# acoustic-warfare/zybo-rt-sampler-image-detection

Measured on AMD Instinct MI355X. Metric: beam-steered frames/sec (64 mics x 256 samples x 101x101 angles), higher is better.
Workload: dtype f32

## Files before the change

zybo-rt-sampler-image-detection_amd/csrc/das_kernels.hip:

```cpp
#include "das_kernels.h"

#include <algorithm>
#include <type_traits>

namespace bf {

namespace {

constexpr int kWave = 64;

struct KArgs {
    long long miso_row;
    int n_mics, m_total, n_samples, n_taps;
    int dir_begin, dir_end, image_stride, image_origin;
    int lead, row_stride, mic_chunk, n_chunks, tile_dirs, n_tiles;
    int scratch_off, srow, pbw;
    int n_is_pow2;
    float inv_n;
    int n_frames;
    int wg_frames, frame_inner;
    long long digest_h_off;
    long long digest_t_off;
};

// ... 1387 lines not shown
    const int f1 = two ? f0 + 1 : f0;
    const int tile_begin = a.dir_begin + tile * a.tile_dirs;
    if (tile_begin >= a.dir_end) return;
    const int tile_end = min(tile_begin + a.tile_dirs, a.dir_end);
    const int M = a.n_mics, N = a.n_samples;
    const int n_half = M / HC;
    const float* __restrict__ sig0 = signals + (size_t)f0 * a.m_total * N;
    const float* __restrict__ sig1 = signals + (size_t)f1 * a.m_total * N;
    float* __restrict__ img0 = images + (size_t)f0 * a.image_stride;
    float* __restrict__ img1 = images + (size_t)f1 * a.image_stride;
    const int32_t* __restrict__ dig = reinterpret_cast<const int32_t*>(taps);

    const int vmic = (lane < n_half) ? mics[lane * HC + (wave >> 1)] : 0;
    auto fetch = [&](int h) -> float4 {
        const int mic = (h < kWave) ? __builtin_amdgcn_readlane(vmic, h) : mics[h * HC + (wave >> 1)];
        const float* src = ((wave & 1) ? sig1 : sig0) + (size_t)mic * N;
        float4 v = make_float4(0.f, 0.f, 0.f, 0.f);
        if (4 * lane < N) v = *reinterpret_cast<const float4*>(src + 4 * lane);
        return v;
    };
    auto stage = [&](int h, const float4 v, bool wipe) {
        float* row0 = lds + (((h & 1) * W) + wave) * G::kSlot;
        const float py = dpp_prev(v.y), pz = dpp_prev(v.z), pw = dpp_prev(v.w);
        write_copies<C>(row0, RS, LEAD, lane, v, py, pz, pw);
        if (wipe) {
            static_assert((LEAD >> 2) * C <= kWave, "one lane per prefix quad");
            constexpr int PQ = LEAD >> 2;
            if (lane < PQ * C) reinterpret_cast<float4*>(row0 + (lane / PQ) * RS)[lane % PQ] = make_float4(0.f, 0.f, 0.f, 0.f);
        }
    };

    float4 st = fetch(0);
    const int lb = 16 * lane + (int)(unsigned)(size_t)((__attribute__((address_space(3))) char*)lds);
    BF_STAMP_DECL

    for (int g0 = tile_begin; g0 < tile_end; g0 += kGroup) {
        f32x2 acc[DW][2][2];
#pragma unroll
        for (int j = 0; j < DW; ++j)
#pragma unroll
            for (int f = 0; f < 2; ++f) { acc[j][f][0] = f32x2{0.0f, 0.0f}; acc[j][f][1] = f32x2{0.0f, 0.0f}; }

        BF_STAMP(7);
        __syncthreads();
        BF_STAMP(1);
        stage(0, st, true);
        st = fetch(1);
        BF_STAMP(2);
        __syncthreads();
        BF_STAMP(3);

        for (int h = 0; h < n_half; ++h) {
            if (h + 1 < n_half) {
                stage(h + 1, st, h == 0);
                if (h + 2 < n_half) st = fetch(h + 2);
                else if (g0 + kGroup < tile_end) st = fetch(0);
                BF_STAMP(2);
            }
            const int dw0 = g0 + wave * DW;
            if (dw0 < tile_end) {
                const size_t grp = (size_t)(dw0 - a.dir_begin) / DW;
                const int32_t* __restrict__ et = dig + (grp * M + (size_t)h * HC) * DW;
                struct Entries { int e[DW]; };
                auto request = [&](Entries& t, int m) {
#pragma unroll
                    for (int j = 0; j < DW; ++j) t.e[j] = et[m * DW + j];
                };
                Entries E[3];
                Quad S0, S1;
                S0.lo = S0.hi = S1.lo = S1.hi = f32x2{0.0f, 0.0f};
                request(E[0], 0);
                request(E[1], 1);
                auto mic = [&](int m, auto kc) {
                    constexpr int K = decltype(kc)::value, K2 = (K + 2) % 3;
                    const Entries& cur = E[K];
                    pair_pad_first(acc, S0, S1, cur.e[0], cur.e[1], lb);
                    request(E[K2], m + 2);
                    pair_pad_rest(acc, S0, S1, cur.e, lb);
                };
                using I0 = std::integral_constant<int, 0>; using I1 = std::integral_constant<int, 1>; using I2 = std::integral_constant<int, 2>;
                static_assert(HC == 8, "eight mics: two trips of three and two more");
#pragma unroll 1
                for (int t = 0; t < 2; ++t) {
                    mic(0, I0{}); mic(1, I1{}); mic(2, I2{});
                    et += 3 * DW;
                }
                mic(0, I0{});
                mic(1, I1{});
            }
            BF_STAMP(0);
            __syncthreads();
            BF_STAMP(h + 1 < n_half ? 3 : 4);
        }

#pragma unroll
        for (int f = 0; f < 2; ++f) {
            if (f == 1) {
                __syncthreads();
                BF_STAMP(4);
            }
            auto park = [&](auto mul_c) {
#pragma unroll
                for (int j = 0; j < DW; ++j) {
                    float* row = lds + (wave * DW + j) * kPark;
                    const f32x2 a0 = acc[j][f][0], a1 = acc[j][f][1];
                    float o0, o1, o2, o3;
                    if constexpr (decltype(mul_c)::value) {
                        o0 = a0.x * a.inv_n; o1 = a0.y * a.inv_n; o2 = a1.x * a.inv_n; o3 = a1.y * a.inv_n;
                    } else {
                        float fm = (float)M;
                        asm volatile("" : "+v"(fm));
                        o0 = a0.x / fm; o1 = a0.y / fm; o2 = a1.x / fm; o3 = a1.y / fm;
                    }
                    reinterpret_cast<float4*>(row)[lane] = make_float4(o0 * o0, o1 * o1, o2 * o2, o3 * o3);
                }
            };
            if (__builtin_expect(a.n_is_pow2, 1)) park(std::true_type{}); else park(std::false_type{});
            BF_STAMP(5);
            __syncthreads();
            BF_STAMP(6);
            const int g = wave * kWave + lane;
            const int d = g0 + g;
            if (g < kGroup && d < tile_end && (f == 0 || two)) {
                const float* row = lds + g * kPark;
                const float4* row4 = reinterpret_cast<const float4*>(row);
                float sum = 0.0f;
                int k = 0;
                for (; k + 32 <= N; k += 32) {
                    float4 v[8];
#pragma unroll
                    for (int u = 0; u < 8; ++u) v[u] = row4[(k >> 2) + u];
#pragma unroll
                    for (int u = 0; u < 8; ++u) { sum += v[u].x; sum += v[u].y; sum += v[u].z; sum += v[u].w; }
                }
                for (; k < N; ++k) sum += row[k];
                (f == 0 ? img0 : img1)[d - a.image_origin] = sum / (float)N;
            }
        }
    }
    BF_STAMP(7);
    BF_STAMP_FLUSH;
}
#undef BF_P_ACC
#undef BF_P_PAD_STEP
#undef BF_P_PAD_READ
#undef BF_P_ADDR
#undef BF_P_CHECK
#undef BF_P_STUB

struct Pair2Geo {
    static constexpr int kC = 2, kLead = Geo<1>::kLead, kRs = 2 * Geo<1>::kRs, kMc = 16, kHalf = 8;
    static constexpr int kSlot = 2 * kC * kRs;
    static constexpr int kDoff = kC * kRs * 4;
};

#define BF_I_ACC(n, j) [a##n##0] "+v"(acc[j][0]), [a##n##1] "+v"(acc[j][1]), [a##n##2] "+v"(acc[j][2]), [a##n##3] "+v"(acc[j][3])
#define BF_I_READ                                                                                   \
    "ds_read_b128 v[96:99], v120\n\tds_read_b128 v[100:103], v120 offset:1024\n\t"                   \
    "ds_read_b128 v[104:107], v120 offset:%[g0]\n\tds_read_b128 v[108:111], v120 offset:%[g1]\n\ts_waitcnt lgkmcnt(0)\n\t"
#define BF_I_STEP(n, h, mods)                                                                       \
    "v_pk_fma_f32 v[112:113], %[" #h "], v[104:105], v[96:97] " mods "\n\tv_pk_fma_f32 v[114:115], %[" #h "], v[106:107], v[98:99] " mods "\n\t" \
    "v_pk_fma_f32 v[116:117], %[" #h "], v[108:109], v[100:101] " mods "\n\tv_pk_fma_f32 v[118:119], %[" #h "], v[110:111], v[102:103] " mods "\n\t" \
    "v_pk_add_f32 %[a" #n "0], %[a" #n "0], v[112:113]\n\tv_pk_add_f32 %[a" #n "1], %[a" #n "1], v[114:115]\n\t" \
    "v_pk_add_f32 %[a" #n "2], %[a" #n "2], v[116:117]\n\tv_pk_add_f32 %[a" #n "3], %[a" #n "3], v[118:119]\n\t"
#define BF_I_FIRST(h, mods)                                                                         \
    "ds_read_b128 v[96:99], v120\n\tds_read_b128 v[104:107], v120 offset:%[g0]\n\t"                \
    "ds_read_b128 v[100:103], v120 offset:1024\n\tds_read_b128 v[108:111], v120 offset:%[g1]\n\ts_waitcnt lgkmcnt(2)\n\t" \
    "v_pk_fma_f32 v[112:113], %[" #h "], v[104:105], v[96:97] " mods "\n\tv_pk_fma_f32 v[114:115], %[" #h "], v[106:107], v[98:99] " mods "\n\t" \
    "v_pk_add_f32 %[a00], %[a00], v[112:113]\n\tv_pk_add_f32 %[a01], %[a01], v[114:115]\n\ts_waitcnt lgkmcnt(0)\n\t" \
    "v_pk_fma_f32 v[116:117], %[" #h "], v[108:109], v[100:101] " mods "\n\tv_pk_fma_f32 v[118:119], %[" #h "], v[110:111], v[102:103] " mods "\n\t" \
    "v_pk_add_f32 %[a02], %[a02], v[116:117]\n\tv_pk_add_f32 %[a03], %[a03], v[118:119]\n\t"
#define BF_I_EVEN "op_sel_hi:[0,1,1]"
#define BF_I_ODD "op_sel:[1,0,0] op_sel_hi:[1,1,1]"
#define BF_I_CHECK(n, ep, ec) "s_cmp_lg_u32 %[" #ec "], %[" #ep "]\n\ts_cbranch_scc1 .Lr" #n "_%=\n.Lb" #n "_%=:\n\t"
#define BF_I_STUB(n, ec) ".Lr" #n "_%=:\n\tv_add_u32 v120, %[" #ec "], %[lb]\n\t" BF_I_READ "s_branch .Lb" #n "_%=\n"
#define BF_I_CLOB "v96", "v97", "v98", "v99", "v100", "v101", "v102", "v103", "v104", "v105", "v106", "v107", "v108", "v109", "v110", "v111", "v112", \
                  "v113", "v114", "v115", "v116", "v117", "v118", "v119", "v120"

__device__ __forceinline__ void pair2_first(f32x2 (&acc)[8][4], int e0, unsigned long long h01, int lbase)
{
    using G = Pair2Geo;
    asm volatile("v_add_u32 v120, %[e0], %[lb]\n\t" BF_I_FIRST(h01, BF_I_EVEN) ";BF_S1_END"
                 : BF_I_ACC(0, 0) : [e0] "s"(e0), [h01] "s"(h01), [lb] "v"(lbase), [g0] "n"(G::kDoff), [g1] "n"(G::kDoff + 1024) : BF_I_CLOB);
}
__device__ __forceinline__ void pair2_rest(f32x2 (&acc)[8][4], const int (&e)[8], const unsigned long long (&hp)[4], int lbase)
{
    using G = Pair2Geo;
    asm volatile(";BF_S2_BEGIN\n\t"
                 BF_I_CHECK(1, e0, e1) BF_I_STEP(1, h01, BF_I_ODD) BF_I_CHECK(2, e1, e2) BF_I_STEP(2, h23, BF_I_EVEN)
                 BF_I_CHECK(3, e2, e3) BF_I_STEP(3, h23, BF_I_ODD) BF_I_CHECK(4, e3, e4) BF_I_STEP(4, h45, BF_I_EVEN)
                 BF_I_CHECK(5, e4, e5) BF_I_STEP(5, h45, BF_I_ODD) BF_I_CHECK(6, e5, e6) BF_I_STEP(6, h67, BF_I_EVEN)
                 BF_I_CHECK(7, e6, e7) BF_I_STEP(7, h67, BF_I_ODD)
                 ".subsection 1\n" BF_I_STUB(1, e1) BF_I_STUB(2, e2) BF_I_STUB(3, e3) BF_I_STUB(4, e4) BF_I_STUB(5, e5) BF_I_STUB(6, e6) BF_I_STUB(7, e7)
                 "\t.subsection 0"
                 : BF_I_ACC(1, 1), BF_I_ACC(2, 2), BF_I_ACC(3, 3), BF_I_ACC(4, 4), BF_I_ACC(5, 5), BF_I_ACC(6, 6), BF_I_ACC(7, 7)
                 : [e0] "s"(e[0]), [e1] "s"(e[1]), [e2] "s"(e[2]), [e3] "s"(e[3]), [e4] "s"(e[4]), [e5] "s"(e[5]), [e6] "s"(e[6]), [e7] "s"(e[7]), [lb] "v"(lbase),
                   [h01] "s"(hp[0]), [h23] "s"(hp[1]), [h45] "s"(hp[2]), [h67] "s"(hp[3]), [g0] "n"(G::kDoff), [g1] "n"(G::kDoff + 1024)
                 : "scc", BF_I_CLOB);
}
#undef BF_I_ACC
#undef BF_I_READ
#undef BF_I_FIRST
#undef BF_I_STEP
#undef BF_I_EVEN
#undef BF_I_ODD
#undef BF_I_CHECK
#undef BF_I_STUB
#undef BF_I_CLOB

template <int ALGO>
__global__ void __launch_bounds__(1024, 4) das_pair2_kernel(BF_TABLE_PARAMS, KArgs a)
{
    static_assert(ALGO == ALGO_LERP, "das_pair2_kernel: lerp (pad runs das_pair_kernel)");
    using G = Pair2Geo;
    constexpr int C = G::kC, RS = G::kRs, LEAD = G::kLead, HC = G::kHalf, W = 16, DW = 8, kGroup = DW * W, kPark = Geo<1>::kPark;
    extern __shared__ __attribute__((aligned(16))) float lds[];
    const int lane_ = threadIdx.x & (kWave - 1), lane = lane_;
    const int wave = __builtin_amdgcn_readfirstlane((int)(threadIdx.x >> 6));
    int tile, fpair;
    tile_and_frame(a, &tile, &fpair);
    const int f0 = 2 * fpair;
    const bool two = f0 + 1 < a.n_frames;
    const int f1 = two ? f0 + 1 : f0;
    const int tile_begin = a.dir_begin + tile * a.tile_dirs;
    if (tile_begin >= a.dir_end) return;
    const int tile_end = min(tile_begin + a.tile_dirs, a.dir_end);
    const int M = a.n_mics, N = a.n_samples;
    const int n_half = M / HC;
    const float* __restrict__ sig0 = signals + (size_t)f0 * a.m_total * N;
    const float* __restrict__ sig1 = signals + (size_t)f1 * a.m_total * N;
    float* __restrict__ img0 = images + (size_t)f0 * a.image_stride;
    float* __restrict__ img1 = images + (size_t)f1 * a.image_stride;
    const int32_t* __restrict__ dig = reinterpret_cast<const int32_t*>(taps);

    const int my_mic = wave & 7, part = wave >> 3;
    const int vmic = (lane < n_half) ? mics[lane * HC + my_mic] : 0;
    struct Staged2 { float4 v0, v1; };
    auto fetch = [&](int h) -> Staged2 {
        const int mic = (h < kWave) ? __builtin_amdgcn_readlane(vmic, h) : mics[h * HC + my_mic];
        Staged2 st;
        st.v0 = make_float4(0.f, 0.f, 0.f, 0.f);
        st.v1 = st.v0;
        if (4 * lane < N) {
            unsigned voff = 16u * (unsigned)lane;
            asm volatile("" : "+v"(voff));
            const char* r0 = reinterpret_cast<const char*>(sig0 + (size_t)mic * N);
            const char* r1 = reinterpret_cast<const char*>(sig1 + (size_t)mic * N);
            st.v0 = *reinterpret_cast<const float4*>(r0 + voff);
            st.v1 = *reinterpret_cast<const float4*>(r1 + voff);
        }
        return st;
    };
    auto write_row = [&](float* row, const float4 x0, const float4 x1, float p0, float p1, bool shifted, int lane) {
        float4* q = reinterpret_cast<float4*>(row + 2 * LEAD) + 2 * lane;
        if (!shifted) {
            q[0] = make_float4(x0.x, x1.x, x0.y, x1.y);
            q[1] = make_float4(x0.z, x1.z, x0.w, x1.w);
        } else {
            q[0] = make_float4(p0, p1, x0.x, x1.x);
            q[1] = make_float4(x0.y, x1.y, x0.z, x1.z);
        }
    };
    auto stage = [&](int h, const Staged2& st, bool wipe) {
        int lane = lane_;
        asm volatile("" : "+v"(lane));
        float* slot = lds + ((h & 1) * HC + my_mic) * G::kSlot;
        float4 x0 = st.v0, x1 = st.v1;
        float* rows = slot + part * C * RS;
        if (part == 1) {
            const float n0 = dpp_next(x0.x), n1 = dpp_next(x1.x);
            x0 = make_float4(x0.y - x0.x, x0.z - x0.y, x0.w - x0.z, n0 - x0.w);
            x1 = make_float4(x1.y - x1.x, x1.z - x1.y, x1.w - x1.z, n1 - x1.w);
        }
        const float p0 = dpp_prev(x0.w), p1 = dpp_prev(x1.w);
        write_row(rows, x0, x1, p0, p1, false, lane);
        write_row(rows + RS, x0, x1, p0, p1, true, lane);
        if (wipe) {
            constexpr int PQ = LEAD >> 1;
            static_assert(2 * PQ <= kWave, "one lane per prefix quad of two rows");
            if (lane < 2 * PQ) reinterpret_cast<float4*>(rows + (lane / PQ) * RS)[lane % PQ] = make_float4(0.f, 0.f, 0.f, 0.f);
        }
    };

    BF_STAMP_DECL
    Staged2 st = fetch(0);
    const int lb = 16 * lane + (int)(unsigned)(size_t)((__attribute__((address_space(3))) char*)lds);

    for (int g0 = tile_begin; g0 < tile_end; g0 += kGroup) {
        f32x2 acc[DW][4];
#pragma unroll
        for (int j = 0; j < DW; ++j)
#pragma unroll
            for (int q = 0; q < 4; ++q) acc[j][q] = f32x2{0.0f, 0.0f};

        BF_STAMP(7);
        __syncthreads();
        BF_STAMP(1);
        stage(0, st, true);
        st = fetch(1 % n_half);
        BF_STAMP(2);
        __syncthreads();
        BF_STAMP(3);

        const int dw0 = g0 + wave * DW;
        const bool busy = dw0 < tile_end;
        const size_t grp = busy ? (size_t)(dw0 - a.dir_begin) / DW : 0;
        for (int h = 0; h < n_half; ++h) {
            if (h + 1 < n_half) {
                stage(h + 1, st, h == 0);
                if (h + 2 < n_half) st = fetch(h + 2);
                else if (g0 + kGroup < tile_end) st = fetch(0);
                BF_STAMP(2);
            }
            if (busy) {
                const int32_t* __restrict__ et = dig + (grp * M + (size_t)h * HC) * DW;
                const float* __restrict__ ht = reinterpret_cast<const float*>(dig) + a.digest_h_off + (grp * M + (size_t)h * HC) * DW;
                struct Entries { int e[DW]; unsigned long long hp[DW / 2]; };
                auto request = [&](Entries& t, int m) {
#pragma unroll
                    for (int j = 0; j < DW; ++j) t.e[j] = et[m * DW + j];
#pragma unroll
                    for (int j = 0; j < DW / 2; ++j) t.hp[j] = *reinterpret_cast<const unsigned long long*>(ht + m * DW + 2 * j);
                };
                Entries E[3];
                request(E[0], 0);
                request(E[1], 1);
                auto mic = [&](int m, auto kc) {
                    constexpr int K = decltype(kc)::value, K2 = (K + 2) % 3;
                    const Entries& cur = E[K];
                    pair2_first(acc, cur.e[0], cur.hp[0], lb);
                    request(E[K2], m + 2);
                    pair2_rest(acc, cur.e, cur.hp, lb);
                };
                using I0 = std::integral_constant<int, 0>; using I1 = std::integral_constant<int, 1>; using I2 = std::integral_constant<int, 2>;
                static_assert(HC == 8, "eight mics: two trips of three and two more");
#pragma unroll 1
                for (int t = 0; t < 2; ++t) {
                    mic(0, I0{}); mic(1, I1{}); mic(2, I2{});
                    et += 3 * DW; ht += 3 * DW;
                }
                mic(0, I0{});
                mic(1, I1{});
                __builtin_amdgcn_s_waitcnt(0xC07F);
            }
            BF_STAMP(0);
            __syncthreads();
            BF_STAMP(h + 1 < n_half ? 3 : 4);
        }

#pragma unroll
        for (int f = 0; f < 2; ++f) {
            if (f == 1) {
                __syncthreads();
                BF_STAMP(4);
            }
            auto park = [&](auto mul_c) __attribute__((always_inline)) {
#pragma unroll
                for (int j = 0; j < DW; ++j) {
                    float* row = lds + (wave * DW + j) * kPark;
                    const float x0 = f == 0 ? acc[j][0].x : acc[j][0].y, x1 = f == 0 ? acc[j][1].x : acc[j][1].y;
                    const float x2 = f == 0 ? acc[j][2].x : acc[j][2].y, x3 = f == 0 ? acc[j][3].x : acc[j][3].y;
                    float o0, o1, o2, o3;
                    if constexpr (decltype(mul_c)::value) {
                        o0 = x0 * a.inv_n; o1 = x1 * a.inv_n; o2 = x2 * a.inv_n; o3 = x3 * a.inv_n;
                    } else {
                        float fm = (float)M;
                        asm volatile("" : "+v"(fm));
                        o0 = x0 / fm; o1 = x1 / fm; o2 = x2 / fm; o3 = x3 / fm;
                    }
                    reinterpret_cast<float2*>(row)[lane] = make_float2(o0 * o0, o1 * o1);
                    reinterpret_cast<float2*>(row + 128)[lane] = make_float2(o2 * o2, o3 * o3);
                }
            };
            if (__builtin_expect(a.n_is_pow2, 1)) park(std::true_type{}); else park(std::false_type{});
            BF_STAMP(5);
            __syncthreads();
            BF_STAMP(6);
            int lane_o = lane;
            asm volatile("" : "+v"(lane_o));
            const int g = wave * kWave + lane_o;
            const int d = g0 + g;
            if (g < kGroup && d < tile_end && (f == 0 || two)) {
                const float* row = lds + g * kPark;
                const float4* row4 = reinterpret_cast<const float4*>(row);
                float sum = 0.0f;
                int k = 0;
                for (; k + 32 <= N; k += 32) {
                    float4 v[8];
#pragma unroll
                    for (int u = 0; u < 8; ++u) v[u] = row4[(k >> 2) + u];
#pragma unroll
                    for (int u = 0; u < 8; ++u) { sum += v[u].x; sum += v[u].y; sum += v[u].z; sum += v[u].w; }
                }
                for (; k < N; ++k) sum += row[k];
                (f == 0 ? img0 : img1)[d - a.image_origin] = sum / (float)N;
            }
        }
    }
    BF_STAMP(7);
    BF_STAMP_FLUSH;
}

struct HybridGeo {
    static constexpr int kC = 2, kLead = Geo<1>::kLead, kRs = 2 * Geo<1>::kRsFir;
    static constexpr int kHalf = 16, kMc = 2 * kHalf;
    static constexpr int kSlot = kC * kRs;
};

struct HybridMasks { unsigned long long m[4]; };
#define BF_H_MASKS                                                                                          \
    "s_lshl_b64 %[m0], -1, %[ng]\n\t"                                                                       \
    "s_lshr_b32 %[t], %[ng], 8\n\ts_lshl_b64 %[m1], -1, %[t]\n\t"                                            \
    "s_lshr_b32 %[t], %[ng], 16\n\ts_lshl_b64 %[m2], -1, %[t]\n\t"                                           \
    "s_lshr_b32 %[t], %[ng], 24\n\ts_lshl_b64 %[m3], -1, %[t]\n\t"
#define BF_H_READS                                                                                          \
    "ds_read_b128 %[q0], %[ad] offset:0\n\tds_read_b128 %[q1], %[ad] offset:16\n\tds_read_b128 %[q2], %[ad] offset:32\n\t" \
    "ds_read_b128 %[q3], %[ad] offset:48\n\tds_read_b128 %[q4], %[ad] offset:64\n\tds_read_b128 %[q5], %[ad] offset:80\n\t"
#define BF_H_QOPS [q0] "+v"(Q[0]), [q1] "+v"(Q[1]), [q2] "+v"(Q[2]), [q3] "+v"(Q[3]), [q4] "+v"(Q[4]), [q5] "+v"(Q[5])
__device__ __forceinline__ void hybrid_window(f32x4 (&Q)[6], HybridMasks& k, int ep, int ec, int ng, int lbase)
{
    int ad, t;
    asm volatile("s_cmp_lg_u32 %[ec], %[ep]\n\ts_cbranch_scc1 .Lr_%=\n.Lb_%=:\n\t"
                 ".subsection 1\n.Lr_%=:\n\tv_add_u32 %[ad], %[ec], %[lb]\n\t" BF_H_READS BF_H_MASKS
                 "s_waitcnt lgkmcnt(0)\n\ts_branch .Lb_%=\n\t.subsection 0"
                 : BF_H_QOPS, [ad] "=&v"(ad), [m0] "+s"(k.m[0]), [m1] "+s"(k.m[1]), [m2] "+s"(k.m[2]), [m3] "+s"(k.m[3]), [t] "=&s"(t)
                 : [ep] "s"(ep), [ec] "s"(ec), [ng] "s"(ng), [lb] "v"(lbase)
                 : "scc");
}
__device__ __forceinline__ void hybrid_window_first(f32x4 (&Q)[6], HybridMasks& k, int ec, int ng, int lbase)
{
    int ad, t;
    asm volatile("v_add_u32 %[ad], %[ec], %[lb]\n\t" BF_H_READS BF_H_MASKS "s_waitcnt lgkmcnt(0)"
                 : BF_H_QOPS, [ad] "=&v"(ad), [m0] "=&s"(k.m[0]), [m1] "=&s"(k.m[1]), [m2] "=&s"(k.m[2]), [m3] "=&s"(k.m[3]), [t] "=&s"(t)
                 : [ec] "s"(ec), [ng] "s"(ng), [lb] "v"(lbase)
                 : "scc");
}
#undef BF_H_MASKS
#undef BF_H_READS
#undef BF_H_QOPS

#define BF_H_E(j, hh, w) "v_pk_fma_f32 %[o" #j "], %[" #hh "], %[w" #w "], %[o" #j "] op_sel_hi:[0,1,1]\n\t"
#define BF_H_O(j, hh, w) "v_pk_fma_f32 %[o" #j "], %[" #hh "], %[w" #w "], %[o" #j "] op_sel:[1,0,0] op_sel_hi:[1,1,1]\n\t"
#define BF_H_OUT(j, w0, w1, w2, w3, w4, w5, w6, w7)                                                          \
    BF_H_E(j, h01, w0) BF_H_O(j, h01, w1) BF_H_E(j, h23, w2) BF_H_O(j, h23, w3) BF_H_E(j, h45, w4) BF_H_O(j, h45, w5) BF_H_E(j, h67, w6) BF_H_O(j, h67, w7)
__device__ __forceinline__ void hybrid_step(f32x2 (&o)[4], const f32x4 (&Q)[6], const unsigned long long (&h)[4], const HybridMasks& k)
{
    const f32x2 w0 = __builtin_shufflevector(Q[0], Q[0], 0, 1), w1 = __builtin_shufflevector(Q[0], Q[0], 2, 3);
    const f32x2 w2 = __builtin_shufflevector(Q[1], Q[1], 0, 1), w3 = __builtin_shufflevector(Q[1], Q[1], 2, 3);
    const f32x2 w4 = __builtin_shufflevector(Q[2], Q[2], 0, 1), w5 = __builtin_shufflevector(Q[2], Q[2], 2, 3);
    const f32x2 w6 = __builtin_shufflevector(Q[3], Q[3], 0, 1), w7 = __builtin_shufflevector(Q[3], Q[3], 2, 3);
    const f32x2 w8 = __builtin_shufflevector(Q[4], Q[4], 0, 1), w9 = __builtin_shufflevector(Q[4], Q[4], 2, 3);
    const f32x2 w10 = __builtin_shufflevector(Q[5], Q[5], 0, 1);
    asm volatile(
        "s_mov_b64 exec, %[m0]\n\t"
        BF_H_OUT(0, 0, 1, 2, 3, 4, 5, 6, 7)
        "s_mov_b64 exec, %[m1]\n\t"
        BF_H_OUT(1, 1, 2, 3, 4, 5, 6, 7, 8)
        "s_mov_b64 exec, %[m2]\n\t"
        BF_H_OUT(2, 2, 3, 4, 5, 6, 7, 8, 9)
        "s_mov_b64 exec, %[m3]\n\t"
        BF_H_OUT(3, 3, 4, 5, 6, 7, 8, 9, 10)
        "s_mov_b64 exec, -1"
        : [o0] "+v"(o[0]), [o1] "+v"(o[1]), [o2] "+v"(o[2]), [o3] "+v"(o[3])
        : [h01] "s"(h[0]), [h23] "s"(h[1]), [h45] "s"(h[2]), [h67] "s"(h[3]), [m0] "s"(k.m[0]), [m1] "s"(k.m[1]), [m2] "s"(k.m[2]), [m3] "s"(k.m[3]),
          [w0] "v"(w0), [w1] "v"(w1), [w2] "v"(w2), [w3] "v"(w3), [w4] "v"(w4), [w5] "v"(w5), [w6] "v"(w6), [w7] "v"(w7), [w8] "v"(w8), [w9] "v"(w9),
          [w10] "v"(w10));
}
__device__ __forceinline__ void fir_naive_step(f32x2 (&o)[4], const f32x4 (&Q)[6], const unsigned long long (&h)[4])
{
    const f32x2 w0 = __builtin_shufflevector(Q[0], Q[0], 0, 1), w1 = __builtin_shufflevector(Q[0], Q[0], 2, 3);
    const f32x2 w2 = __builtin_shufflevector(Q[1], Q[1], 0, 1), w3 = __builtin_shufflevector(Q[1], Q[1], 2, 3);
    const f32x2 w4 = __builtin_shufflevector(Q[2], Q[2], 0, 1), w5 = __builtin_shufflevector(Q[2], Q[2], 2, 3);
    const f32x2 w6 = __builtin_shufflevector(Q[3], Q[3], 0, 1), w7 = __builtin_shufflevector(Q[3], Q[3], 2, 3);
    const f32x2 w8 = __builtin_shufflevector(Q[4], Q[4], 0, 1), w9 = __builtin_shufflevector(Q[4], Q[4], 2, 3);
    const f32x2 w10 = __builtin_shufflevector(Q[5], Q[5], 0, 1);
    asm volatile(
        BF_H_OUT(0, 0, 1, 2, 3, 4, 5, 6, 7) BF_H_OUT(1, 1, 2, 3, 4, 5, 6, 7, 8) BF_H_OUT(2, 2, 3, 4, 5, 6, 7, 8, 9) BF_H_OUT(3, 3, 4, 5, 6, 7, 8, 9, 10)
        : [o0] "+v"(o[0]), [o1] "+v"(o[1]), [o2] "+v"(o[2]), [o3] "+v"(o[3])
        : [h01] "s"(h[0]), [h23] "s"(h[1]), [h45] "s"(h[2]), [h67] "s"(h[3]),
          [w0] "v"(w0), [w1] "v"(w1), [w2] "v"(w2), [w3] "v"(w3), [w4] "v"(w4), [w5] "v"(w5), [w6] "v"(w6), [w7] "v"(w7), [w8] "v"(w8), [w9] "v"(w9),
          [w10] "v"(w10));
}
#define BF_V_MUL(p, hh, w, MODS) "v_pk_mul_f32 %[" #p "], %[" #hh "], %[w" #w "] " MODS "\n\t"
#define BF_V_OUT(j, w0, w1, w2, w3, w4, w5, w6, w7)                                                                             \
    BF_V_MUL(p0, h01, w0, "op_sel_hi:[0,1]") BF_V_MUL(p1, h01, w1, "op_sel:[1,0] op_sel_hi:[1,1]")                                \
    BF_V_MUL(p2, h23, w2, "op_sel_hi:[0,1]") BF_V_MUL(p3, h23, w3, "op_sel:[1,0] op_sel_hi:[1,1]")                                \
    BF_V_MUL(p4, h45, w4, "op_sel_hi:[0,1]") BF_V_MUL(p5, h45, w5, "op_sel:[1,0] op_sel_hi:[1,1]")                                \
    BF_V_MUL(p6, h67, w6, "op_sel_hi:[0,1]") BF_V_MUL(p7, h67, w7, "op_sel:[1,0] op_sel_hi:[1,1]")                                \
    "v_pk_add_f32 %[p0], %[p0], %[p4]\n\tv_pk_add_f32 %[p1], %[p1], %[p5]\n\tv_pk_add_f32 %[p2], %[p2], %[p6]\n\tv_pk_add_f32 %[p3], %[p3], %[p7]\n\t" \
    "v_pk_add_f32 %[p0], %[p0], %[p2]\n\tv_pk_add_f32 %[p1], %[p1], %[p3]\n\tv_pk_add_f32 %[p0], %[p0], %[p1]\n\t"                   \
    "v_pk_add_f32 %[o" #j "], %[o" #j "], %[p0]\n\t"
__device__ __forceinline__ void fir_vec_step(f32x2 (&o)[4], const f32x4 (&Q)[6], const unsigned long long (&h)[4])
{
    const f32x2 w0 = __builtin_shufflevector(Q[0], Q[0], 0, 1), w1 = __builtin_shufflevector(Q[0], Q[0], 2, 3);
    const f32x2 w2 = __builtin_shufflevector(Q[1], Q[1], 0, 1), w3 = __builtin_shufflevector(Q[1], Q[1], 2, 3);
    const f32x2 w4 = __builtin_shufflevector(Q[2], Q[2], 0, 1), w5 = __builtin_shufflevector(Q[2], Q[2], 2, 3);
    const f32x2 w6 = __builtin_shufflevector(Q[3], Q[3], 0, 1), w7 = __builtin_shufflevector(Q[3], Q[3], 2, 3);
    const f32x2 w8 = __builtin_shufflevector(Q[4], Q[4], 0, 1), w9 = __builtin_shufflevector(Q[4], Q[4], 2, 3);
    const f32x2 w10 = __builtin_shufflevector(Q[5], Q[5], 0, 1);
    f32x2 p0, p1, p2, p3, p4, p5, p6, p7;
    asm volatile(
        BF_V_OUT(0, 0, 1, 2, 3, 4, 5, 6, 7) BF_V_OUT(1, 1, 2, 3, 4, 5, 6, 7, 8) BF_V_OUT(2, 2, 3, 4, 5, 6, 7, 8, 9) BF_V_OUT(3, 3, 4, 5, 6, 7, 8, 9, 10)
        : [o0] "+v"(o[0]), [o1] "+v"(o[1]), [o2] "+v"(o[2]), [o3] "+v"(o[3]), [p0] "=&v"(p0), [p1] "=&v"(p1), [p2] "=&v"(p2), [p3] "=&v"(p3),
          [p4] "=&v"(p4), [p5] "=&v"(p5), [p6] "=&v"(p6), [p7] "=&v"(p7)
        : [h01] "s"(h[0]), [h23] "s"(h[1]), [h45] "s"(h[2]), [h67] "s"(h[3]),
          [w0] "v"(w0), [w1] "v"(w1), [w2] "v"(w2), [w3] "v"(w3), [w4] "v"(w4), [w5] "v"(w5), [w6] "v"(w6), [w7] "v"(w7), [w8] "v"(w8), [w9] "v"(w9),
          [w10] "v"(w10));
}
#undef BF_V_MUL
#undef BF_V_OUT
#undef BF_H_OUT
#undef BF_H_E
#undef BF_H_O
__device__ __forceinline__ void fir_window_first(f32x4 (&Q)[6], int ec, int lbase)
{
    int ad;
    asm volatile("v_add_u32 %[ad], %[ec], %[lb]\n\t"
                 "ds_read_b128 %[q0], %[ad] offset:0\n\tds_read_b128 %[q1], %[ad] offset:16\n\tds_read_b128 %[q2], %[ad] offset:32\n\t"
                 "ds_read_b128 %[q3], %[ad] offset:48\n\tds_read_b128 %[q4], %[ad] offset:64\n\tds_read_b128 %[q5], %[ad] offset:80\n\t"
                 "s_waitcnt lgkmcnt(0)"
                 : [q0] "=&v"(Q[0]), [q1] "=&v"(Q[1]), [q2] "=&v"(Q[2]), [q3] "=&v"(Q[3]), [q4] "=&v"(Q[4]), [q5] "=&v"(Q[5]), [ad] "=&v"(ad)
                 : [ec] "s"(ec), [lb] "v"(lbase));
}

template <int ALGO>
__global__ void __launch_bounds__(1024, 4) das_hybrid_pair_kernel(BF_TABLE_PARAMS, KArgs a)
{
    constexpr bool kHybrid = ALGO == ALGO_HYBRID;
    using G = HybridGeo;
    constexpr int C = G::kC, RS = G::kRs, LEAD = G::kLead, HC = G::kHalf, W = 16, DW = 8, kGroup = DW * W, kPark = Geo<1>::kPark;
    extern __shared__ __attribute__((aligned(16))) float lds[];
    const int lane = threadIdx.x & (kWave - 1);
    const int wave = __builtin_amdgcn_readfirstlane((int)(threadIdx.x >> 6));
    int tile, fpair;
    tile_and_frame(a, &tile, &fpair);
    const int f0 = 2 * fpair;
    const bool two = f0 + 1 < a.n_frames;
    const int f1 = two ? f0 + 1 : f0;
    const int tile_begin = a.dir_begin + tile * a.tile_dirs;
    if (tile_begin >= a.dir_end) return;
    const int tile_end = min(tile_begin + a.tile_dirs, a.dir_end);
    const int M = a.n_mics, N = a.n_samples;
    const int n_half = M / HC;
    const float* __restrict__ sig0 = signals + (size_t)f0 * a.m_total * N;
    const float* __restrict__ sig1 = signals + (size_t)f1 * a.m_total * N;
    float* __restrict__ img0 = images + (size_t)f0 * a.image_stride;
    float* __restrict__ img1 = images + (size_t)f1 * a.image_stride;
    const int32_t* __restrict__ dig = reinterpret_cast<const int32_t*>(frac);
// ... 478 lines not shown
            for (int sg = 0; sg < NSEG; ++sg) { acc[j][sg][0] = f32x2{0.0f, 0.0f}; acc[j][sg][1] = f32x2{0.0f, 0.0f}; }

        __syncthreads();
        if (my_seg == 0) wipe_prefix();
        StagedL st = fetch_next();
        stage(0, st);
        st = fetch_next();
        const int dw0 = g0 + wave * DW;
        const bool busy = dw0 < tile_end;
        const size_t grp = busy ? (size_t)(dw0 - a.dir_begin) / DW : 0;
        const int32_t* __restrict__ et = dig + grp * M * DW;
        const float* __restrict__ ht = reinterpret_cast<const float*>(dig) + a.digest_h_off + grp * M * DW;
        struct Entries { int e[DW]; unsigned long long hp[DW / 2]; };
        auto request = [&](Entries& t, int m) {
#pragma unroll
            for (int j = 0; j < DW; ++j) t.e[j] = et[m * DW + j];
#pragma unroll
            for (int j = 0; j < DW / 2; ++j) {
                t.hp[j] = 0;
                if constexpr (kLerp) t.hp[j] = *reinterpret_cast<const unsigned long long*>(ht + m * DW + 2 * j);
            }
        };
        constexpr int KE = HC == 4 ? 4 : 3;
        Entries E[KE];
        request(E[0], 0);
        request(E[1], 1);
        __syncthreads();

        for (int h = 0; h < n_half; ++h) {
            if (h + 1 < n_half) {
                stage(h + 1, st);
                if (h + 2 < n_half) st = fetch_next();
            }
            if (busy) {
                auto mic = [&](int m, auto kc, auto pc) {
                    constexpr int K = decltype(kc)::value, K2 = (K + 2) % KE, POS = decltype(pc)::value;
                    const Entries& cur = E[K];
                    if constexpr (kLerp) {
                        if constexpr (POS == 0) long_lerp_first<NSEG>(acc, cur.e[0], cur.hp[0], lb);
                        else long_lerp_cont<NSEG>(acc, cur.hp[0]);
                        __builtin_amdgcn_s_waitcnt(0xC07F);
                        request(E[K2], m + 2);
                        if constexpr (POS == HC - 1) long_lerp_rest<NSEG, false>(acc, cur.e, cur.hp, lb, 0);
                        else long_lerp_rest<NSEG, true>(acc, cur.e, cur.hp, lb, E[(K + 1) % KE].e[0]);
                    } else {
                        if constexpr (POS == 0) long_pad_first<NSEG>(acc, cur.e[0], lb);
                        else long_pad_cont<NSEG>(acc);
                        __builtin_amdgcn_s_waitcnt(0xC07F);
                        request(E[K2], m + 2);
                        if constexpr (POS == HC - 1) long_pad_rest<NSEG, false>(acc, cur.e, lb, 0);
                        else long_pad_rest<NSEG, true>(acc, cur.e, lb, E[(K + 1) % KE].e[0]);
                    }
                };
                using I0 = std::integral_constant<int, 0>; using I1 = std::integral_constant<int, 1>; using I2 = std::integral_constant<int, 2>;
                using I3 = std::integral_constant<int, 3>;
                const int m0 = h * HC;
                if constexpr (HC == 4) {
                    mic(m0 + 0, I0{}, I0{}); mic(m0 + 1, I1{}, I1{}); mic(m0 + 2, I2{}, I2{}); mic(m0 + 3, I3{}, I3{});
                } else {
                    using I4 = std::integral_constant<int, 4>; using I5 = std::integral_constant<int, 5>; using I6 = std::integral_constant<int, 6>;
                    using I7 = std::integral_constant<int, 7>;
                    mic(m0 + 0, I0{}, I0{}); mic(m0 + 1, I1{}, I1{}); mic(m0 + 2, I2{}, I2{}); mic(m0 + 3, I0{}, I3{});
                    mic(m0 + 4, I1{}, I4{}); mic(m0 + 5, I2{}, I5{}); mic(m0 + 6, I0{}, I6{}); mic(m0 + 7, I1{}, I7{});
                    const Entries t = E[0]; E[0] = E[2]; E[1] = t;
                }
            }
            __syncthreads();
        }

        const int pw_waves = a.pbw;
        for (int w0 = 0; w0 < W; w0 += pw_waves) {
            if (w0 > 0) __syncthreads();
            if (wave >= w0 && wave < w0 + pw_waves) {
                auto park = [&](auto mul_c) __attribute__((always_inline)) {
#pragma unroll
                    for (int j = 0; j < DW; ++j) {
                        float* row = lds + ((wave - w0) * DW + j) * kPark;
#pragma unroll
                        for (int sg = 0; sg < NSEG; ++sg) {
                            f32x2 a0 = acc[j][sg][0], a1 = acc[j][sg][1];
                            asm volatile("" : "+v"(a0), "+v"(a1));
                            float o0, o1, o2, o3;
                            if constexpr (decltype(mul_c)::value) {
                                o0 = a0.x * a.inv_n; o1 = a0.y * a.inv_n; o2 = a1.x * a.inv_n; o3 = a1.y * a.inv_n;
                            } else {
                                float fm = (float)M;
                                asm volatile("" : "+v"(fm));
                                o0 = a0.x / fm; o1 = a0.y / fm; o2 = a1.x / fm; o3 = a1.y / fm;
                                __builtin_amdgcn_sched_barrier(0);
                            }
                            reinterpret_cast<float2*>(row + 256 * sg)[lane] = make_float2(o0 * o0, o1 * o1);
                            reinterpret_cast<float2*>(row + 256 * sg + 128)[lane] = make_float2(o2 * o2, o3 * o3);
                        }
                    }
                };
                if (__builtin_expect(a.n_is_pow2, 1)) park(std::true_type{}); else park(std::false_type{});
            }
            __syncthreads();
            const int g = wave * kWave + lane;
            const int d = g0 + w0 * DW + g;
            if (g < pw_waves * DW && d < tile_end) {
                const float* row = lds + g * kPark;
                const float4* row4 = reinterpret_cast<const float4*>(row);
                float sum = 0.0f;
                int k = 0;
                for (; k + 32 <= N; k += 32) {
                    float4 v[8];
#pragma unroll
                    for (int u = 0; u < 8; ++u) v[u] = row4[(k >> 2) + u];
#pragma unroll
                    for (int u = 0; u < 8; ++u) { sum += v[u].x; sum += v[u].y; sum += v[u].z; sum += v[u].w; }
                }
                for (; k < N; ++k) sum += row[k];
                img[d - a.image_origin] = sum / (float)N;
            }
        }
    }
}

}

template <typename K>
static hipError_t refuse_scratch(K kernel, int* cached)
{
    if (*cached < 0) {
        hipFuncAttributes fa{};
        hipError_t e = hipFuncGetAttributes(&fa, reinterpret_cast<const void*>(kernel));
        if (e != hipSuccess) return e;
        *cached = (int)fa.localSizeBytes;
    }
#ifdef BF_STAMPS
    return hipSuccess;
#else
    return *cached != 0 ? hipErrorInvalidDeviceFunction : hipSuccess;
#endif
}

template <int ALGO, int NSEG>
hipError_t launch_copies(const DasLaunch& L, const KArgs& a, const DasPlan& plan, int frames, hipStream_t stream)
{
    const dim3 grid((unsigned)plan.n_tiles * (unsigned)frames);
    const dim3 block((unsigned)plan.waves * kWave);
    constexpr bool kFir = ALGO == ALGO_HYBRID || ALGO == ALGO_FIR_NAIVE || ALGO == ALGO_FIR_VEC;
    constexpr bool kNeedsDigest = ALGO != ALGO_FIR_NAIVE && ALGO != ALGO_FIR_VEC;
    if (kNeedsDigest && L.tab.digest == nullptr) return hipErrorInvalidValue;
    if (kFir && L.n_taps != 8) return hipErrorInvalidValue;
    if constexpr (!kFir && NSEG == 1) {
        if (plan.nf == 2) {
            constexpr bool kLerp = ALGO == ALGO_LERP;
            using PG = std::conditional_t<kLerp, copies::Pair2Geo, copies::PairGeo>;
            if (L.tab.digest_direct || plan.waves != copies::kWaves || plan.mic_chunk != PG::kMc || plan.row_stride != PG::kRs ||
                plan.lead != PG::kLead || plan.interleaved != (kLerp ? 1 : 0) || (L.n_mics % 16) != 0)
                return hipErrorInvalidValue;
            auto kernel = [] { if constexpr (kLerp) return copies::das_pair2_kernel<ALGO>; else return copies::das_pair_kernel<ALGO>; }();
            hipError_t e = hipFuncSetAttribute(reinterpret_cast<const void*>(kernel), hipFuncAttributeMaxDynamicSharedMemorySize, (int)plan.lds_bytes);
            if (e != hipSuccess) return e;
            static int pair_scratch = -1;
            if ((e = refuse_scratch(kernel, &pair_scratch)) != hipSuccess) return e;
            const dim3 pair_grid((unsigned)plan.n_tiles * (unsigned)((frames + 1) / 2));
            hipLaunchKernelGGL(kernel, pair_grid, block, plan.lds_bytes, stream, L.signals, L.images, L.mics, L.tab.whole, L.tab.frac,
                               reinterpret_cast<const float*>(L.tab.digest), a);
            return hipGetLastError();
        }
    }
    if constexpr (kFir) {
        if (plan.nf == 2) {
            using HG = copies::HybridGeo;
            if (L.tab.digest == nullptr || plan.waves != copies::kWaves || plan.mic_chunk != HG::kMc || plan.row_stride != HG::kRs ||
                plan.lead != HG::kLead || (L.n_mics % 16) != 0 || L.n_taps != 8)
                return hipErrorInvalidValue;
            auto kernel = copies::das_hybrid_pair_kernel<ALGO>;
            hipError_t e = hipFuncSetAttribute(reinterpret_cast<const void*>(kernel), hipFuncAttributeMaxDynamicSharedMemorySize, (int)plan.lds_bytes);
            if (e != hipSuccess) return e;
            static int hybrid_scratch = -1;
            if ((e = refuse_scratch(kernel, &hybrid_scratch)) != hipSuccess) return e;
            const dim3 pair_grid((unsigned)plan.n_tiles * (unsigned)((frames + 1) / 2));
            hipLaunchKernelGGL(kernel, pair_grid, block, plan.lds_bytes, stream, L.signals, L.images, L.mics, L.tab.whole,
                               reinterpret_cast<const float*>(L.tab.digest), L.tab.taps, a);
            return hipGetLastError();
        }
    }
    if constexpr (!kFir && (NSEG == 2 || NSEG == 4)) {
        if (plan.long_rows) {
            using LG = copies::LongGeo<ALGO, NSEG>;
            if (L.tab.digest == nullptr || L.tab.digest_direct || plan.waves != copies::kWaves || plan.mic_chunk != LG::kMc ||
                (L.n_mics % LG::kHalf) != 0 || plan.dpw != LG::kDw)
                return hipErrorInvalidValue;
            const bool fixed_rs = plan.row_stride == (LG::kLerp ? 2 : 1) * copies::Geo<NSEG>::kRs && plan.lead == copies::Geo<NSEG>::kLead;
            auto kernel = fixed_rs ? copies::das_long_kernel<ALGO, NSEG, copies::Geo<NSEG>::kRs> : copies::das_long_kernel<ALGO, NSEG, 0>;
            hipError_t e = hipFuncSetAttribute(reinterpret_cast<const void*>(kernel), hipFuncAttributeMaxDynamicSharedMemorySize, (int)plan.lds_bytes);
            if (e != hipSuccess) return e;
            static int long_scratch[2] = {-1, -1};
            if ((e = refuse_scratch(kernel, &long_scratch[fixed_rs ? 1 : 0])) != hipSuccess) return e;
            hipLaunchKernelGGL(kernel, grid, block, plan.lds_bytes, stream, L.signals, L.images, L.mics, L.tab.whole, L.tab.frac,
                               reinterpret_cast<const float*>(L.tab.digest), a);
            return hipGetLastError();
        }
    }
    using G = copies::Geo<NSEG>;
    constexpr int kRs = kFir ? G::kRsFir : G::kRs;
    const bool fixed = plan.row_stride == kRs && plan.lead == G::kLead;
    auto kernel = fixed ? copies::das_copies_kernel<ALGO, NSEG, kRs, copies::kWaves> : copies::das_copies_kernel<ALGO, NSEG, 0, copies::kWaves>;
    if constexpr (!kFir && NSEG == 1) {
        if (plan.waves == 8) kernel = fixed ? copies::das_copies_kernel<ALGO, NSEG, kRs, 8> : copies::das_copies_kernel<ALGO, NSEG, 0, 8>;
    }
    bool direct = false;
    if constexpr (!kFir) {
        if (L.tab.digest_direct) {
            if (plan.waves != copies::kWaves) return hipErrorInvalidValue;
            kernel = fixed ? copies::das_copies_kernel<ALGO, NSEG, kRs, copies::kWaves, true> : copies::das_copies_kernel<ALGO, NSEG, 0, copies::kWaves, true>;
            direct = true;
        }
    }
    if (plan.waves != copies::kWaves && !(plan.waves == 8 && !kFir && NSEG == 1)) return hipErrorInvalidValue;
    hipError_t e = hipFuncSetAttribute(reinterpret_cast<const void*>(kernel), hipFuncAttributeMaxDynamicSharedMemorySize, (int)plan.lds_bytes);
    if (e != hipSuccess) return e;
    if constexpr (!kFir && NSEG == 1) if (!direct) {
        static int scratch_bytes[4] = {-1, -1, -1, -1};
        int& sb = scratch_bytes[(fixed ? 1 : 0) + (plan.waves == 8 ? 2 : 0)];
        if (sb < 0) {
            hipFuncAttributes fa{};
            e = hipFuncGetAttributes(&fa, reinterpret_cast<const void*>(kernel));
            if (e != hipSuccess) return e;
            sb = (int)fa.localSizeBytes;
        }
        if (sb != 0) return hipErrorInvalidDeviceFunction;
    }
    const float* dig = reinterpret_cast<const float*>(L.tab.digest);
    hipLaunchKernelGGL(kernel, grid, block, plan.lds_bytes, stream, L.signals, L.images, L.mics, L.tab.whole, kFir ? dig : L.tab.frac,
                       kFir ? L.tab.taps : dig, a);
    return hipGetLastError();
}

template <int ALGO, int NC>
hipError_t launch_nc(const DasLaunch& L, const KArgs& a, const DasPlan& plan, int frames, hipStream_t stream)
{
    constexpr bool kFir = ALGO == ALGO_HYBRID || ALGO == ALGO_FIR_NAIVE || ALGO == ALGO_FIR_VEC;
    if constexpr (!kFir && NC >= 4) {
        return plan.layout == 2 ? launch_copies<ALGO, NC / 4>(L, a, plan, frames, stream) : hipErrorInvalidValue;
    } else {
        if constexpr (NC == 4) {
            if (plan.layout == 2) return launch_copies<ALGO, 1>(L, a, plan, frames, stream);
        }
        auto go = [&](auto kernel) -> hipError_t {
            hipError_t e = hipFuncSetAttribute(reinterpret_cast<const void*>(kernel), hipFuncAttributeMaxDynamicSharedMemorySize,
                                               (int)plan.lds_bytes);
            if (e != hipSuccess) return e;
            hipLaunchKernelGGL(kernel, dim3((unsigned)plan.n_tiles * (unsigned)frames), dim3((unsigned)plan.waves * kWave), plan.lds_bytes, stream,
                               L.signals, L.images, L.mics, L.tab.whole, L.tab.frac, L.tab.taps, a);
            return hipGetLastError();
        };
        switch (plan.dpw) {
            case 1: return go(das_mimo_kernel<ALGO, NC, 1>);
            case 4: return go(das_mimo_kernel<ALGO, NC, 4>);
            default: return hipErrorInvalidValue;
        }
    }
}

template <int ALGO>
hipError_t launch_algo(const DasLaunch& L, const KArgs& a, const DasPlan& plan, int frames, hipStream_t stream)
{
    switch (plan.nc) {
        case 1: return launch_nc<ALGO, 1>(L, a, plan, frames, stream);
        case 2: return launch_nc<ALGO, 2>(L, a, plan, frames, stream);
        case 4: return launch_nc<ALGO, 4>(L, a, plan, frames, stream);
        case 8: return launch_nc<ALGO, 8>(L, a, plan, frames, stream);
        case 16: return launch_nc<ALGO, 16>(L, a, plan, frames, stream);
        default: return hipErrorInvalidValue;
    }
}

struct MisoBatch {
    const int32_t* offsets = nullptr;
    int frames = 1, beams = 1, waves = 1;
    int* status = nullptr;
    long long entries = 0;
    float gain = 0.0f;
    int out_stride = 0;
};

template <int ALGO>
hipError_t launch_miso_algo(const DasLaunch& L, const KArgs& a, const DasPlan& plan, const float* init_dev, float* out_dev, const MisoBatch& B,
                            hipStream_t stream)
{
    const unsigned groups = (unsigned)((B.beams + B.waves - 1) / B.waves);
    const int out_stride = B.out_stride > 0 ? B.out_stride : L.n_samples;
    auto go = [&](auto kernel) -> hipError_t {
        hipError_t e = hipFuncSetAttribute(reinterpret_cast<const void*>(kernel), hipFuncAttributeMaxDynamicSharedMemorySize,
                                           (int)plan.lds_bytes);
        if (e != hipSuccess) return e;
        hipLaunchKernelGGL(kernel, dim3((unsigned)B.frames * groups), dim3((unsigned)B.waves * kWave), plan.lds_bytes, stream, L.signals, L.images, L.mics,
                           L.tab.whole, L.tab.frac, L.tab.taps, init_dev, out_dev, a, B.offsets, B.beams, B.status, B.entries, B.gain, out_stride);
        return hipGetLastError();
    };
    switch (plan.nc) {
        case 1: return go(das_miso_kernel<ALGO, 1>);
        case 2: return go(das_miso_kernel<ALGO, 2>);
        case 4: return go(das_miso_kernel<ALGO, 4>);
        case 8: return go(das_miso_kernel<ALGO, 8>);
        case 16: return go(das_miso_kernel<ALGO, 16>);
        default: return hipErrorInvalidValue;
    }
}

long long grouped_entries_for_args(const DasLaunch& L, const DasPlan& plan)
{
    const long long groups = ((long long)(L.dir_end - L.dir_begin) + plan.dpw - 1) / plan.dpw;
    return groups * L.n_mics * plan.dpw;
}

KArgs make_args(const DasLaunch& L, const DasPlan& plan)
{
// ... 374 lines not shown
```

Baseline: 136,400.

## Split final reduction into half-row passes across four waves for both frames

The final per-direction sum over samples is restructured. Instead of parking a full row per frame and reducing each frame in its own pass with two waves, both frames' data are parked as 128-sample half rows, padded to 132 floats to avoid bank conflicts, and aliased over the staging LDS. Four waves reduce them, two per frame, accumulating across two passes. The reduction loop is also software-pipelined with double-buffered float4 loads and sched barriers. This spreads the tail reduction over more waves and hides LDS latency, at the cost of more complex indexing. The N<=256 half split relies on the sample count assumption.

New measurement: 137,300 (median of 6 runs). No clear change (+0.7%).

```diff
diff --git a/zybo-rt-sampler-image-detection_amd/csrc/das_kernels.hip b/zybo-rt-sampler-image-detection_amd/csrc/das_kernels.hip
--- a/zybo-rt-sampler-image-detection_amd/csrc/das_kernels.hip
+++ b/zybo-rt-sampler-image-detection_amd/csrc/das_kernels.hip
@@ -1563,6 +1563,7 @@
     static constexpr int kC = 2, kLead = Geo<1>::kLead, kRs = 2 * Geo<1>::kRs, kMc = 16, kHalf = 8;
     static constexpr int kSlot = 2 * kC * kRs;
     static constexpr int kDoff = kC * kRs * 4;
+    static constexpr int kHalfRow = 128 + 4;
 };
 
 #define BF_I_ACC(n, j) [a##n##0] "+v"(acc[j][0]), [a##n##1] "+v"(acc[j][1]), [a##n##2] "+v"(acc[j][2]), [a##n##3] "+v"(acc[j][3])
@@ -1624,7 +1625,8 @@
 {
     static_assert(ALGO == ALGO_LERP, "das_pair2_kernel: lerp (pad runs das_pair_kernel)");
     using G = Pair2Geo;
-    constexpr int C = G::kC, RS = G::kRs, LEAD = G::kLead, HC = G::kHalf, W = 16, DW = 8, kGroup = DW * W, kPark = Geo<1>::kPark;
+    constexpr int C = G::kC, RS = G::kRs, LEAD = G::kLead, HC = G::kHalf, W = 16, DW = 8, kGroup = DW * W, kHalfRow = G::kHalfRow;
+    static_assert(2 * kGroup * kHalfRow <= G::kMc * G::kSlot, "the half rows of both frames' chains alias the staged mics");
     extern __shared__ __attribute__((aligned(16))) float lds[];
     const int lane_ = threadIdx.x & (kWave - 1), lane = lane_;
     const int wave = __builtin_amdgcn_readfirstlane((int)(threadIdx.x >> 6));
@@ -1759,52 +1761,81 @@
             BF_STAMP(h + 1 < n_half ? 3 : 4);
         }
 
-#pragma unroll
-        for (int f = 0; f < 2; ++f) {
-            if (f == 1) {
+        const bool chain_wave = wave < 4 && g0 + (wave & 1) * kWave < tile_end && (wave < 2 || two);
+        float sum = 0.0f;
+#pragma unroll
+        for (int p = 0; p < 2; ++p) {
+            if (p == 1) {
+                BF_STAMP(7);
                 __syncthreads();
                 BF_STAMP(4);
             }
             auto park = [&](auto mul_c) __attribute__((always_inline)) {
+                int lane = lane_;
+                asm volatile("" : "+v"(lane));
 #pragma unroll
                 for (int j = 0; j < DW; ++j) {
-                    float* row = lds + (wave * DW + j) * kPark;
-                    const float x0 = f == 0 ? acc[j][0].x : acc[j][0].y, x1 = f == 0 ? acc[j][1].x : acc[j][1].y;
-                    const float x2 = f == 0 ? acc[j][2].x : acc[j][2].y, x3 = f == 0 ? acc[j][3].x : acc[j][3].y;
+                    float* row = lds + (wave * DW + j) * kHalfRow;
+                    const f32x2 u = acc[j][2 * p], v = acc[j][2 * p + 1];
                     float o0, o1, o2, o3;
                     if constexpr (decltype(mul_c)::value) {
-                        o0 = x0 * a.inv_n; o1 = x1 * a.inv_n; o2 = x2 * a.inv_n; o3 = x3 * a.inv_n;
+                        o0 = u.x * a.inv_n; o1 = v.x * a.inv_n; o2 = u.y * a.inv_n; o3 = v.y * a.inv_n;
                     } else {
                         float fm = (float)M;
                         asm volatile("" : "+v"(fm));
-                        o0 = x0 / fm; o1 = x1 / fm; o2 = x2 / fm; o3 = x3 / fm;
+                        o0 = u.x / fm; o1 = v.x / fm; o2 = u.y / fm; o3 = v.y / fm;
                     }
                     reinterpret_cast<float2*>(row)[lane] = make_float2(o0 * o0, o1 * o1);
-                    reinterpret_cast<float2*>(row + 128)[lane] = make_float2(o2 * o2, o3 * o3);
+                    reinterpret_cast<float2*>(row + kGroup * kHalfRow)[lane] = make_float2(o2 * o2, o3 * o3);
                 }
             };
             if (__builtin_expect(a.n_is_pow2, 1)) park(std::true_type{}); else park(std::false_type{});
             BF_STAMP(5);
             __syncthreads();
             BF_STAMP(6);
-            int lane_o = lane;
-            asm volatile("" : "+v"(lane_o));
-            const int g = wave * kWave + lane_o;
-            const int d = g0 + g;
-            if (g < kGroup && d < tile_end && (f == 0 || two)) {
-                const float* row = lds + g * kPark;
-                const float4* row4 = reinterpret_cast<const float4*>(row);
-                float sum = 0.0f;
-                int k = 0;
-                for (; k + 32 <= N; k += 32) {
-                    float4 v[8];
-#pragma unroll
-                    for (int u = 0; u < 8; ++u) v[u] = row4[(k >> 2) + u];
-#pragma unroll
-                    for (int u = 0; u < 8; ++u) { sum += v[u].x; sum += v[u].y; sum += v[u].z; sum += v[u].w; }
-                }
-                for (; k < N; ++k) sum += row[k];
-                (f == 0 ? img0 : img1)[d - a.image_origin] = sum / (float)N;
+            if (chain_wave) {
+                int lane_o = lane;
+                asm volatile("" : "+v"(lane_o));
+                const float4* row4 = reinterpret_cast<const float4*>(lds + (wave * kWave + lane_o) * kHalfRow);
+                const int np = p == 0 ? min(N, 128) : max(N - 128, 0);
+                const int nb = np >> 4;
+                auto load = [&](float4 (&b)[4], int i) __attribute__((always_inline)) {
+#pragma unroll
+                    for (int u = 0; u < 4; ++u) b[u] = row4[4 * i + u];
+                    __builtin_amdgcn_sched_barrier(0);
+                };
+                auto add = [&](const float4 (&b)[4]) __attribute__((always_inline)) {
+#pragma unroll
+                    for (int u = 0; u < 4; ++u) { sum += b[u].x; sum += b[u].y; sum += b[u].z; sum += b[u].w; }
+                    __builtin_amdgcn_sched_barrier(0);
+                };
+                if (nb > 0) {
+                    float4 b0[4], b1[4];
+                    int i = 0;
+                    load(b0, 0);
+#pragma unroll 1
+                    for (; i + 2 < nb; i += 2) {
+                        load(b1, i + 1);
+                        add(b0);
+                        load(b0, i + 2);
+                        add(b1);
+                    }
+                    if (i + 1 < nb) {
+                        load(b1, i + 1);
+                        add(b0);
+                        add(b1);
+                    } else {
+                        add(b0);
+                    }
+                }
+                for (int q = 4 * nb; 4 * q < np; ++q) {
+                    const float4 v = row4[q];
+                    sum += v.x; sum += v.y; sum += v.z; sum += v.w;
+                }
+                if (p == 1) {
+                    const int d = g0 + (wave & 1) * kWave + lane_o;
+                    if (d < tile_end) (wave < 2 ? img0 : img1)[d - a.image_origin] = sum / (float)N;
+                }
             }
         }
     }
```

## Replace per-half workgroup barriers with LDS counter-based producer/consumer signaling in pair2 kernel

Applied to the files above, without the earlier changes.

Replaces the __syncthreads between mic-half stages in the lerp pair2 kernel with per-parity LDS counters. Waves atomically increment these counters when they finish staging or consuming, and spin-wait on them with s_sleep, so staging of the next half can overlap with other waves still computing. A bounded spin with a give-up flag that poisons results with NaN guards against deadlock. Extra LDS bytes are reserved for the counters. The cost is spin overhead, LDS atomic traffic, and subtle ordering risk.

Result: slower. 136,300 before, 124,800 after (-8.4%).

```diff
diff --git a/zybo-rt-sampler-image-detection_amd/csrc/das_kernels.hip b/zybo-rt-sampler-image-detection_amd/csrc/das_kernels.hip
--- a/zybo-rt-sampler-image-detection_amd/csrc/das_kernels.hip
+++ b/zybo-rt-sampler-image-detection_amd/csrc/das_kernels.hip
@@ -1563,6 +1563,9 @@
     static constexpr int kC = 2, kLead = Geo<1>::kLead, kRs = 2 * Geo<1>::kRs, kMc = 16, kHalf = 8;
     static constexpr int kSlot = 2 * kC * kRs;
     static constexpr int kDoff = kC * kRs * 4;
+    static constexpr int kImage = kMc * kSlot * 4;
+    static constexpr int kCtrBytes = 32;
+    static constexpr int kSpinMax = 1 << 20;
 };
 
 #define BF_I_ACC(n, j) [a##n##0] "+v"(acc[j][0]), [a##n##1] "+v"(acc[j][1]), [a##n##2] "+v"(acc[j][2]), [a##n##3] "+v"(acc[j][3])
@@ -1619,6 +1622,28 @@
 #undef BF_I_STUB
 #undef BF_I_CLOB
 
+__device__ __forceinline__ int pair2_peek(int addr)
+{
+    int t, got;
+    asm volatile("v_mov_b32 %[t], %[ad]\n\tds_read_b32 %[t], %[t]\n\ts_waitcnt lgkmcnt(0)\n\tv_readfirstlane_b32 %[g], %[t]"
+                 : [t] "=&v"(t), [g] "=s"(got) : [ad] "s"(addr) : "memory");
+    return got;
+}
+__device__ __forceinline__ void pair2_signal(int addr)
+{
+    int t, one;
+    unsigned long long ex;
+    asm volatile("s_waitcnt lgkmcnt(0)\n\ts_mov_b64 %[ex], exec\n\ts_mov_b64 exec, 1\n\tv_mov_b32 %[t], %[ad]\n\tv_mov_b32 %[o], 1\n\t"
+                 "ds_add_u32 %[t], %[o]\n\ts_mov_b64 exec, %[ex]"
+                 : [t] "=&v"(t), [o] "=&v"(one), [ex] "=&s"(ex) : [ad] "s"(addr) : "memory");
+}
+__device__ __forceinline__ void pair2_give_up(int addr)
+{
+    int t, one;
+    asm volatile("v_mov_b32 %[t], %[ad]\n\tv_mov_b32 %[o], 1\n\tds_write_b32 %[t], %[o]\n\ts_waitcnt lgkmcnt(0)"
+                 : [t] "=&v"(t), [o] "=&v"(one) : [ad] "s"(addr) : "memory");
+}
+
 template <int ALGO>
 __global__ void __launch_bounds__(1024, 4) das_pair2_kernel(BF_TABLE_PARAMS, KArgs a)
 {
@@ -1697,6 +1722,20 @@
     Staged2 st = fetch(0);
     const int lb = 16 * lane + (int)(unsigned)(size_t)((__attribute__((address_space(3))) char*)lds);
 
+    const int ctr = (int)(unsigned)(size_t)((__attribute__((address_space(3))) char*)lds) + G::kImage;
+    if (threadIdx.x < G::kCtrBytes / 4) lds[G::kImage / 4 + threadIdx.x] = 0.0f;
+    int base = 0;
+    auto wait_for = [&](int addr, int target) __attribute__((always_inline)) {
+        if (__builtin_expect(pair2_peek(addr) - target < 0, 0)) {
+            for (int trips = 0; ; ++trips) {
+                if (pair2_peek(ctr + 16) != 0) break;
+                if (trips == G::kSpinMax) { pair2_give_up(ctr + 16); break; }
+                __builtin_amdgcn_s_sleep(2);
+                if (pair2_peek(addr) - target >= 0) break;
+            }
+        }
+    };
+
     for (int g0 = tile_begin; g0 < tile_end; g0 += kGroup) {
         f32x2 acc[DW][4];
 #pragma unroll
@@ -1708,6 +1747,7 @@
         __syncthreads();
         BF_STAMP(1);
         stage(0, st, true);
+        pair2_signal(ctr);
         st = fetch(1 % n_half);
         BF_STAMP(2);
         __syncthreads();
@@ -1717,13 +1757,23 @@
         const bool busy = dw0 < tile_end;
         const size_t grp = busy ? (size_t)(dw0 - a.dir_begin) / DW : 0;
         for (int h = 0; h < n_half; ++h) {
-            if (h + 1 < n_half) {
-                stage(h + 1, st, h == 0);
-                if (h + 2 < n_half) st = fetch(h + 2);
-                else if (g0 + kGroup < tile_end) st = fetch(0);
-                BF_STAMP(2);
-            }
+            const int par = (h & 1) << 2;
+            auto midpoint = [&]() __attribute__((always_inline)) {
+                if (h + 1 < n_half) {
+                    BF_STAMP(0);
+                    wait_for(ctr + 12 - par, base + (((h + 1) >> 1) << 4));
+                    BF_STAMP(3);
+                    stage(h + 1, st, h == 0);
+                    pair2_signal(ctr + 4 - par);
+                    if (h + 2 < n_half) st = fetch(h + 2);
+                    else if (g0 + kGroup < tile_end) st = fetch(0);
+                    BF_STAMP(2);
+                }
+            };
+            if (!busy) midpoint();
             if (busy) {
+                wait_for(ctr + par, base + (((h >> 1) + 1) << 4));
+                BF_STAMP(3);
                 const int32_t* __restrict__ et = dig + (grp * M + (size_t)h * HC) * DW;
                 const float* __restrict__ ht = reinterpret_cast<const float*>(dig) + a.digest_h_off + (grp * M + (size_t)h * HC) * DW;
                 struct Entries { int e[DW]; unsigned long long hp[DW / 2]; };
@@ -1749,14 +1799,23 @@
                 for (int t = 0; t < 2; ++t) {
                     mic(0, I0{}); mic(1, I1{}); mic(2, I2{});
                     et += 3 * DW; ht += 3 * DW;
+                    if (t == 0) midpoint();
                 }
                 mic(0, I0{});
                 mic(1, I1{});
                 __builtin_amdgcn_s_waitcnt(0xC07F);
             }
             BF_STAMP(0);
-            __syncthreads();
-            BF_STAMP(h + 1 < n_half ? 3 : 4);
+            pair2_signal(ctr + 8 + par);
+        }
+        base += n_half << 3;
+        __syncthreads();
+        BF_STAMP(4);
+        if (__builtin_expect(pair2_peek(ctr + 16) != 0, 0)) {
+#pragma unroll
+            for (int j = 0; j < DW; ++j)
+#pragma unroll
+                for (int q = 0; q < 4; ++q) acc[j][q] = f32x2{__builtin_nanf(""), __builtin_nanf("")};
         }
 
 #pragma unroll
@@ -2589,13 +2648,18 @@
             if (L.tab.digest_direct || plan.waves != copies::kWaves || plan.mic_chunk != PG::kMc || plan.row_stride != PG::kRs ||
                 plan.lead != PG::kLead || plan.interleaved != (kLerp ? 1 : 0) || (L.n_mics % 16) != 0)
                 return hipErrorInvalidValue;
+            size_t lds_bytes = plan.lds_bytes;
+            if constexpr (kLerp) {
+                if (plan.lds_bytes != (size_t)PG::kImage) return hipErrorInvalidValue;
+                lds_bytes += PG::kCtrBytes;
+            }
             auto kernel = [] { if constexpr (kLerp) return copies::das_pair2_kernel<ALGO>; else return copies::das_pair_kernel<ALGO>; }();
-            hipError_t e = hipFuncSetAttribute(reinterpret_cast<const void*>(kernel), hipFuncAttributeMaxDynamicSharedMemorySize, (int)plan.lds_bytes);
+            hipError_t e = hipFuncSetAttribute(reinterpret_cast<const void*>(kernel), hipFuncAttributeMaxDynamicSharedMemorySize, (int)lds_bytes);
             if (e != hipSuccess) return e;
             static int pair_scratch = -1;
             if ((e = refuse_scratch(kernel, &pair_scratch)) != hipSuccess) return e;
             const dim3 pair_grid((unsigned)plan.n_tiles * (unsigned)((frames + 1) / 2));
-            hipLaunchKernelGGL(kernel, pair_grid, block, plan.lds_bytes, stream, L.signals, L.images, L.mics, L.tab.whole, L.tab.frac,
+            hipLaunchKernelGGL(kernel, pair_grid, block, lds_bytes, stream, L.signals, L.images, L.mics, L.tab.whole, L.tab.frac,
                                reinterpret_cast<const float*>(L.tab.digest), a);
             return hipGetLastError();
         }
```
